# Picovoice/koala

Measured on AMD Instinct MI355X. Metric: 16 kHz frames/sec (batch 4096 streams per GPU), higher is better.
Workload: dtype bf16; 1 GPU; BASELINE configs[2]: batch=4096 streams/GPU x 64 frames/call, bf16 mask GEMMs on MFMA + fp32 FFT; streams_per_gpu=4096, frames_per_call=64, global_streams=4096, parallelism=streams sharded over 1 GPU(s), no data-path collective

## Files before the change

### koala_amd/csrc/kns_device.hpp

```cpp
#pragma once

#include <hip/hip_runtime.h>
#include <stdint.h>
#include <stdlib.h>

#include "kns_kernels.h"

namespace kns {

#ifdef KNS_TIMING
static __device__ unsigned long long g_kns_timing[8 * 16];
#define KNS_STAMP(i) do { if (blockIdx.x == 0 && (threadIdx.x & 63) == 0 && t == 5) g_kns_timing[(threadIdx.x >> 6) * 16 + (i)] = __builtin_amdgcn_s_memtime(); } while (0)
#define KNS_STAMP_AT(i, step) do { if (blockIdx.x == 0 && (threadIdx.x & 63) == 0 && t == (step)) g_kns_timing[(threadIdx.x >> 6) * 16 + (i)] = __builtin_amdgcn_s_memtime(); } while (0)
#define KNS_WSTAMP(i) do { if (dbg_stamp && (threadIdx.x & 63) == 0 && mt == m0 + 1) g_kns_timing[role * 16 + (i)] = __builtin_amdgcn_s_memtime(); } while (0)
#else
#define KNS_WSTAMP(i) do { } while (0)
#define KNS_STAMP(i) do { } while (0)
#define KNS_STAMP_AT(i, step) do { } while (0)
#endif

typedef float f32x4 __attribute__((ext_vector_type(4)));
typedef __bf16 bf16x8 __attribute__((ext_vector_type(8)));
typedef _Float16 f16x4 __attribute__((ext_vector_type(4)));

// ... 76 lines not shown
    __builtin_amdgcn_fence(__ATOMIC_RELEASE, "wavefront");
    __builtin_amdgcn_wave_barrier();
    __builtin_amdgcn_fence(__ATOMIC_ACQUIRE, "wavefront");
}


struct PF32 {
    static constexpr int kPrec = kFp32;
    static constexpr int KB = 16, EPL = 4, NPB = 1;
    static constexpr int NBH = 17;
    static constexpr bool kHoldA = false;
    static constexpr int kGruWaves = 1;
    typedef f32x4 frag_t;
    typedef f32x4 gi_t;
    typedef float elem_t;
    static __device__ __forceinline__ f32x4 mma(frag_t a, frag_t b, f32x4 c) {
        c = __builtin_amdgcn_mfma_f32_16x16x4f32(a[0], b[0], c, 0, 0, 0);
        c = __builtin_amdgcn_mfma_f32_16x16x4f32(a[1], b[1], c, 0, 0, 0);
        c = __builtin_amdgcn_mfma_f32_16x16x4f32(a[2], b[2], c, 0, 0, 0);
        c = __builtin_amdgcn_mfma_f32_16x16x4f32(a[3], b[3], c, 0, 0, 0);
        return c;
    }
    static __device__ __forceinline__ void mma2(frag_t a0, frag_t b0, f32x4 &c0, frag_t a1, frag_t b1, f32x4 &c1) {
#pragma unroll
        for (int q = 0; q < 4; ++q) {
            c0 = __builtin_amdgcn_mfma_f32_16x16x4f32(a0[q], b0[q], c0, 0, 0, 0);
            c1 = __builtin_amdgcn_mfma_f32_16x16x4f32(a1[q], b1[q], c1, 0, 0, 0);
        }
    }
    static __device__ __forceinline__ int off(int rc, int kk) { return pack_off_f32(rc, kk); }
    static __device__ __forceinline__ elem_t cvt(float v) { return v; }
    static __device__ __forceinline__ gi_t to_gi(f32x4 v) { return v; }
    static __device__ __forceinline__ f32x4 from_gi(gi_t v) { return v; }
};

struct PBF16 {
    static constexpr int kPrec = kBf16;
    static constexpr int KB = 32, EPL = 8, NPB = 2;
    static constexpr int NBH = 9;
    static constexpr bool kHoldA = true;
    static constexpr int kGruWaves = 1;
    typedef bf16x8 frag_t;
    typedef f16x4 gi_t;
    typedef uint16_t elem_t;
    static __device__ __forceinline__ f32x4 mma(frag_t a, frag_t b, f32x4 c) {
        return __builtin_amdgcn_mfma_f32_16x16x32_bf16(a, b, c, 0, 0, 0);
    }
    static __device__ __forceinline__ void mma2(frag_t a0, frag_t b0, f32x4 &c0, frag_t a1, frag_t b1, f32x4 &c1) {
        c0 = __builtin_amdgcn_mfma_f32_16x16x32_bf16(a0, b0, c0, 0, 0, 0);
        c1 = __builtin_amdgcn_mfma_f32_16x16x32_bf16(a1, b1, c1, 0, 0, 0);
    }
    static __device__ __forceinline__ int off(int rc, int kk) { return pack_off_bf16(rc, kk); }
    static __device__ __forceinline__ elem_t cvt(float v) { return f2bf(v); }
    static __device__ __forceinline__ gi_t to_gi(f32x4 v) { return __builtin_convertvector(v, gi_t); }
    static __device__ __forceinline__ f32x4 from_gi(gi_t v) {
        f32x4 r;
        r[0] = (float) v[0];
        r[1] = (float) v[1];
        r[2] = (float) v[2];
        r[3] = (float) v[3];
        return r;
    }
};


#ifdef KNS_CPX_PACKED
typedef float cpx __attribute__((ext_vector_type(2)));
__device__ __forceinline__ cpx cadd(cpx a, cpx b) { return a + b; }
__device__ __forceinline__ cpx csub(cpx a, cpx b) { return a - b; }
__device__ __forceinline__ cpx cmul(cpx a, cpx w) {
    const cpx t = cpx{a.y, a.y} * cpx{-w.y, w.x};
    return __builtin_elementwise_fma(cpx{a.x, a.x}, w, t);
}
#else
struct alignas(8) cpx {
    float x, y;
};
__device__ __forceinline__ cpx cadd(cpx a, cpx b) { return cpx{a.x + b.x, a.y + b.y}; }
__device__ __forceinline__ cpx csub(cpx a, cpx b) { return cpx{a.x - b.x, a.y - b.y}; }
__device__ __forceinline__ cpx cmul(cpx a, cpx w) {
    return cpx{__builtin_fmaf(a.x, w.x, a.y * -w.y), __builtin_fmaf(a.x, w.y, a.y * w.x)};
}
#endif

__device__ __forceinline__ void radix4(cpx (&v)[4]) {
    cpx a0 = cadd(v[0], v[2]), a1 = csub(v[0], v[2]), a2 = cadd(v[1], v[3]), d = csub(v[1], v[3]);
    cpx a3 = {d.y, -d.x};
    v[0] = cadd(a0, a2);
    v[1] = cadd(a1, a3);
    v[2] = csub(a0, a2);
    v[3] = csub(a1, a3);
}

constexpr int kFftRowBytes = 16 * 17 * 8;
constexpr int kFftWaveBytes = 4 * kFftRowBytes;
// ... 81 lines not shown
    return kns_sigmoid(x);
}
__device__ __forceinline__ float fast_tanh(float x) {
    return 1.0f - 2.0f * __builtin_amdgcn_rcpf(1.0f + __builtin_amdgcn_exp2f(x * 2.88539008177792681f));
}

typedef float f32x2 __attribute__((ext_vector_type(2)));
typedef __bf16 bf16x2 __attribute__((ext_vector_type(2)));

__device__ __forceinline__ __amdgpu_buffer_rsrc_t make_rsrc(const void *base, unsigned bytes) {
    return __builtin_amdgcn_make_buffer_rsrc((void *) base, 0, bytes, 0x00020000);
}
__device__ __forceinline__ bf16x8 buf_load_frag(__amdgpu_buffer_rsrc_t r, unsigned voff, unsigned soff) {
    return __builtin_bit_cast(bf16x8, __builtin_amdgcn_raw_buffer_load_b128(r, voff, soff, 0));
}
__device__ __forceinline__ void buf_store_frag(__amdgpu_buffer_rsrc_t r, unsigned voff, bf16x8 v) {
    typedef unsigned u32x4 __attribute__((ext_vector_type(4)));
    __builtin_amdgcn_raw_buffer_store_b128(__builtin_bit_cast(u32x4, v), r, voff, 0, 0);
}
__device__ __forceinline__ void buf_store_f32x4(__amdgpu_buffer_rsrc_t r, unsigned voff, f32x4 v) {
    typedef unsigned u32x4 __attribute__((ext_vector_type(4)));
    __builtin_amdgcn_raw_buffer_store_b128(__builtin_bit_cast(u32x4, v), r, voff, 0, 0);
}
__device__ __forceinline__ unsigned reset_rows(const unsigned *resets, int pitch, int mt, int t) {
    typedef const __attribute__((address_space(4))) unsigned *cptr_t;
    return __builtin_amdgcn_readfirstlane(((cptr_t) resets)[(size_t) mt * pitch + t]);
}

constexpr int kGiStreamAux = 2;
__device__ __forceinline__ void buf_store_gi(__amdgpu_buffer_rsrc_t r, unsigned voff, unsigned soff, f16x4 v) {
    typedef unsigned u32x2 __attribute__((ext_vector_type(2)));
    __builtin_amdgcn_raw_buffer_store_b64(__builtin_bit_cast(u32x2, v), r, voff, soff, kGiStreamAux);
}

__device__ __forceinline__ f32x2 gate_fma2(f32x2 a, f32x2 b, f32x2 c) {
#ifdef KNS_GATE_UNFUSED
    return a * b + c;
#else
    return __builtin_elementwise_fma(a, b, c);
#endif
}
__device__ __forceinline__ float gate_fma1(float a, float b, float c) {
#ifdef KNS_GATE_UNFUSED
    return a * b + c;
#else
    return __builtin_fmaf(a, b, c);
#endif
}
typedef _Float16 f16x2 __attribute__((ext_vector_type(2)));
__device__ __forceinline__ float opaque_one() {
    float one = 1.0f;
    asm("" : "+v"(one));
    return one;
}
template <int HI>
__device__ __forceinline__ float mix_add(unsigned x, float t, float one) {
    return __builtin_fmaf((float) __builtin_bit_cast(f16x2, x)[HI], one, t);
}
template <int HI>
__device__ __forceinline__ float mix_fma(float a, float b, unsigned x) {
    return __builtin_fmaf(a, b, (float) __builtin_bit_cast(f16x2, x)[HI]);
}

__device__ __forceinline__ float gate_rcp1p_exp2(float y) { return __builtin_amdgcn_rcpf(1.0f + __builtin_amdgcn_exp2f(y)); }
__device__ __forceinline__ f32x4 gate_block_bf16(const unsigned (&pr)[2], const unsigned (&pz)[2], const unsigned (&pn)[2],
                                                 const f32x4 &ar_, const f32x4 &az_, const f32x4 &an_, const f32x4 &hprev) {
// ... 35 lines not shown
```

### koala_amd/csrc/kns_gemm.hip

```cpp
#include "kns_device.hpp"

#include <type_traits>

namespace kns {


constexpr int kPF = 4;

template <class P, int OUT, int kGemmMT>
__global__ __launch_bounds__(256) void gemm_kernel(GemmArgs g) {
    extern __shared__ __attribute__((aligned(16))) char smem[];
    typedef typename P::frag_t frag_t;
    constexpr bool kApack = (OUT == kOutAPlain || OUT == kOutASigmoid);
    constexpr bool kSigmoid = (OUT == kOutMask || OUT == kOutASigmoid);
    constexpr int NU = kApack ? P::NPB : 1;

    const int tid = threadIdx.x, lane = tid & 63;
    const int wave = __builtin_amdgcn_readfirstlane(tid >> 6);
    const int nb = g.nb0 + g.taps * g.nb1;
    const int mt0 = blockIdx.x * kGemmMT;
    const int mcount = min(kGemmMT, g.mtiles - mt0);

    const int units = g.ntiles / NU;
    const int units_per_y = ceil_div(units, (int) gridDim.y);
// ... 50 lines not shown
                    for (int j = 0; j < NU; ++j) bc[j] = bq[p][j];
                    if (blk + kPF < nb)
#pragma unroll
                        for (int j = 0; j < NU; ++j) bq[p][j] = w[((size_t) (nt0 + j) * nb + blk + kPF) * 64 + lane];
#pragma unroll
                    for (int m = 0; m < kGemmMT; ++m) {
                        frag_t a = lds_f[(m * nb + blk) * 64 + lane];
#pragma unroll
                        for (int j = 0; j < NU; ++j) acc[j][m] = P::mma(a, bc[j], acc[j][m]);
                    }
                }
            }
        }

#pragma unroll
        for (int j = 0; j < NU; ++j) {
            const int nt = nt0 + j;
            const int col = nt * 16 + (lane & 15);
            const float bias = g.bias[col];
#pragma unroll
            for (int m = 0; m < kGemmMT; ++m) {
                f32x4 v = acc[j][m];
#pragma unroll
                for (int i = 0; i < 4; ++i) {
                    float x = v[i] + bias;
                    if (kSigmoid) x = head_sigmoid<P>(x);
                    if (kApack && col >= g.n_valid) x = 0.0f;
                    v[i] = x;
                }
                if (!kApack) {
                    if (m < mcount) {
                        const size_t idx = ((size_t) (mt0 + m) * g.ntiles + nt) * 64 + lane;
                        if (OUT == kOutGi)
                            ((typename P::gi_t *) g.out)[idx] = P::to_gi(v);
                        else if (P::kPrec == kBf16)
                            ((f16x4 *) g.out)[idx] = __builtin_convertvector(v, f16x4);
                        else
                            ((f32x4 *) g.out)[idx] = v;
                    }
                } else if (OUT == kOutASigmoid && g.pad_nb) {
                    if (m < mcount && col < g.n_valid) {
                        typename P::elem_t *dst = (typename P::elem_t *) g.out + ((size_t) (mt0 + m) * g.pad_nb + g.pad_blk) * 64 * P::EPL;
#pragma unroll
                        for (int i = 0; i < 4; ++i) dst[P::off((lane >> 4) * 4 + i, g.pad_kk0 + col)] = P::cvt(v[i]);
                    }
                } else {
                    typename P::elem_t *sc = (typename P::elem_t *) (scratch + m * 1024);
#pragma unroll
                    for (int i = 0; i < 4; ++i) sc[P::off((lane >> 4) * 4 + i, j * 16 + (lane & 15))] = P::cvt(v[i]);
                }
            }
        }
        if (kApack && !(OUT == kOutASigmoid && g.pad_nb)) {
            wave_lds_sync();
            const int out_nb = g.ntiles / NU;
            for (int m = 0; m < mcount; ++m) {
                uint4 word = ((const uint4 *) (scratch + m * 1024))[lane];
                ((uint4 *) g.out)[((size_t) (mt0 + m) * out_nb + u) * 64 + lane] = word;
            }
            wave_lds_sync();
        }
    }
}

constexpr int kWs2Waves = 8;
constexpr int kWs2Tiles = 4;

#ifndef WS2_NA
#define WS2_NA 2
#endif
constexpr int kWs2NA = WS2_NA;

template <int NB0, int kWs2Stage>
__global__ __launch_bounds__(64 * kWs2Waves, 2) void gemm_ws2_kernel(GemmArgs g) {
    typedef PBF16 P;
    typedef P::frag_t frag_t;
    constexpr int NB = P::NBH + NB0;
    __shared__ __attribute__((aligned(16))) char smem[2 * kWs2Stage * NB * 1024];
    frag_t *abuf = (frag_t *) smem;

    const int tid = threadIdx.x, lane = tid & 63;
    const int wave = __builtin_amdgcn_readfirstlane(tid >> 6);
    const int colq = lane & 15;
    const int bid = blockIdx.x;
    const int half = (bid >> 3) & 1;
    const int mgroup = (bid >> 4) * 8 + (bid & 7);
    const int mstride = (gridDim.x >> 1) * kWs2Stage;
    const int mlast = mgroup * kWs2Stage + ((g.mtiles - 1 - mgroup * kWs2Stage) / mstride) * mstride;
    const int nt_base = half ? 26 : 0, nt_count = half ? kGateTiles - 26 : 26;
    const frag_t *w = (const frag_t *) g.w;

    int nt[kWs2Tiles];
#pragma unroll
    for (int j = 0; j < kWs2Tiles; ++j) nt[j] = nt_base + (wave + kWs2Waves * j < nt_count ? wave + kWs2Waves * j : 0);
    const bool has4 = wave + kWs2Waves * 3 < nt_count;
    frag_t wr[kWs2Tiles][NB];
    float bias[kWs2Tiles];
#pragma unroll
    for (int j = 0; j < kWs2Tiles; ++j) {
#pragma unroll
        for (int blk = 0; blk < NB; ++blk) wr[j][blk] = w[((size_t) nt[j] * NB + blk) * 64 + lane];
        bias[j] = g.bias[nt[j] * 16 + colq];
    }

    constexpr int kStageBlocks = kWs2Stage * NB;
    constexpr int kFetch = (kStageBlocks + kWs2Waves - 1) / kWs2Waves;
    const unsigned lane16 = lane * 16u, lane8 = lane * 8u;
    unsigned foff[kFetch];
#pragma unroll
    for (int i = 0; i < kFetch; ++i) {
        const int idx = wave + kWs2Waves * i;
        const int m = idx / NB, blk = idx % NB;
        foff[i] = blk < NB0 ? (unsigned) (m * NB0 + blk) * 1024u : (unsigned) (m * P::NBH + (blk - NB0)) * 1024u;
    }
    auto fetch = [&](int i, int mt0) {
        const int blk = (wave + kWs2Waves * i) % NB;
        const __amdgpu_buffer_rsrc_t r =
            blk < NB0 ? make_rsrc((const frag_t *) g.a0 + (size_t) mt0 * NB0 * 64, kWs2Stage * (NB0 ? NB0 : 1) * 1024)
                      : make_rsrc((const frag_t *) g.a1 + (size_t) mt0 * P::NBH * 64, kWs2Stage * P::NBH * 1024);
        return buf_load_frag(r, lane16, foff[i]);
    };
#pragma unroll
    for (int i = 0; i < kFetch; ++i)
        if (wave + kWs2Waves * i < kStageBlocks) abuf[(wave + kWs2Waves * i) * 64 + lane] = fetch(i, mlast);
    __syncthreads();

    auto store_tile = [&](__amdgpu_buffer_rsrc_t out, int j, f32x4 v) {
#pragma unroll
        for (int i = 0; i < 4; ++i) v[i] = v[i] + bias[j];
        buf_store_gi(out, lane8, nt[j] * 512u, P::to_gi(v));
    };

    auto main_loop = [&](auto has4_tag) {
        constexpr bool kHas4 = decltype(has4_tag)::value;
        int cur = 0;
        for (int mt0 = mlast; mt0 >= 0; mt0 -= mstride) {
            const bool more = mt0 - mstride >= 0;
            frag_t stage[kFetch];
#pragma unroll
            for (int i = 0; i < kFetch; ++i)
                if (more && wave + kWs2Waves * i < kStageBlocks) stage[i] = fetch(i, mt0 - mstride);
            constexpr int MP = NB0 < 2 ? 2 : 1;
            static_assert(kWs2Stage % MP == 0, "m-tiles are processed MP at a time");
            const frag_t *ab = abuf + cur * kStageBlocks * 64;
#pragma unroll
            for (int m = 0; m < kWs2Stage; m += MP) {
                f32x4 acc[MP][kWs2Tiles];
                frag_t qa[MP][kWs2NA];
#pragma unroll
                for (int mm = 0; mm < MP; ++mm) {
#pragma unroll
                    for (int c = 0; c < kWs2Tiles; ++c) acc[mm][c] = f32x4{0.f, 0.f, 0.f, 0.f};
#pragma unroll
                    for (int p = 0; p < kWs2NA; ++p) qa[mm][p] = ab[((m + mm) * NB + p) * 64 + lane];
                }
                __builtin_amdgcn_sched_barrier(0);
#pragma unroll
                for (int blk = 0; blk < NB; ++blk) {
#pragma unroll
                    for (int c = 0; c < (kHas4 ? 4 : 3); ++c)
#pragma unroll
                        for (int mm = 0; mm < MP; ++mm) acc[mm][c] = P::mma(qa[mm][blk % kWs2NA], wr[c][blk], acc[mm][c]);
                    if (blk + kWs2NA < NB) {
#pragma unroll
                        for (int mm = 0; mm < MP; ++mm)
                            qa[mm][blk % kWs2NA] = ab[((m + mm) * NB + blk + kWs2NA) * 64 + lane];
                    }
                    __builtin_amdgcn_sched_barrier(0);
                }
                if (m == kWs2Stage - MP) {
#pragma unroll
                    for (int i = 0; i < kFetch; ++i)
                        if (more && wave + kWs2Waves * i < kStageBlocks)
                            abuf[((cur ^ 1) * kStageBlocks + wave + kWs2Waves * i) * 64 + lane] = stage[i];
                }
#pragma unroll
                for (int mm = 0; mm < MP; ++mm) {
                    const __amdgpu_buffer_rsrc_t out =
                        make_rsrc((P::gi_t *) g.out + (size_t) (mt0 + m + mm) * kGateTiles * 64, kGateTiles * 512);
#pragma unroll
                    for (int c = 0; c < (kHas4 ? 4 : 3); ++c) store_tile(out, c, acc[mm][c]);
                }
            }
            __syncthreads();
            cur ^= 1;
        }
    };
    if (has4)
        main_loop(std::true_type{});
    else
        main_loop(std::false_type{});
}

constexpr int kWsrStage = 2;

template <int OUT, int UW>
__global__ __launch_bounds__(512, 2) void gemm_wsr_kernel(GemmArgs g) {
    typedef PBF16 P;
    typedef P::frag_t frag_t;
    constexpr int NB = P::NBH;
    constexpr bool kApack = (OUT == kOutAPlain || OUT == kOutASigmoid);
    constexpr bool kSigmoid = (OUT == kOutMask || OUT == kOutASigmoid);
    constexpr int NU = kApack ? P::NPB : 1;
    __shared__ __attribute__((aligned(16))) char smem[2 * kWsrStage * NB * 1024 + 8 * 1024];
    frag_t *abuf = (frag_t *) smem;
    const int tid = threadIdx.x, lane = tid & 63;
    const int wave = __builtin_amdgcn_readfirstlane(tid >> 6);
    char *scratch = smem + 2 * kWsrStage * NB * 1024 + wave * 1024;
    const int colq = lane & 15;
    const int units = g.ntiles / NU;
    const frag_t *w = (const frag_t *) g.w;

    int unit[UW];
    bool live[UW];
    frag_t wr[UW * NU][NB];
    float bias[UW * NU];
#pragma unroll
    for (int q = 0; q < UW; ++q) {
        live[q] = wave + 8 * q < units;
        unit[q] = live[q] ? wave + 8 * q : 0;
#pragma unroll
        for (int j = 0; j < NU; ++j) {
            const int nt = unit[q] * NU + j;
#pragma unroll
// ... 386 lines not shown
        launch_gemm_mt<P, 2>(a, s);
    else
        launch_gemm_mt<P, 1>(a, s);
}

void launch_gemm(const GemmArgs &a, hipStream_t s) {
    const bool no_ws = (a.dev & kDevGemmGeneric) != 0;
    if (a.precision == kBf16 && a.out_kind == kOutGi && a.ntiles == kGateTiles && a.nb1 == PBF16::NBH && a.nb0 <= 2 && a.taps == 1 &&
        a.mtiles >= 256 && !no_ws) {
        GemmArgs m = a;
        m.mtiles = a.mtiles / 256 * 256;
        const int wgs = a.grid >= 16 && a.grid < 256 ? (a.grid / 16 >= 8 ? 128 : a.grid / 16 >= 4 ? 64 : a.grid / 16 >= 2 ? 32 : 16) : 256;
        const dim3 grid(wgs), block(64 * kWs2Waves);
        if (m.mtiles % 512 == 0) {
            if (a.nb0 == 0)
                hipLaunchKernelGGL((gemm_ws2_kernel<0, 4>), grid, block, 0, s, m);
            else if (a.nb0 == 1)
                hipLaunchKernelGGL((gemm_ws2_kernel<1, 4>), grid, block, 0, s, m);
            else
                hipLaunchKernelGGL((gemm_ws2_kernel<2, 4>), grid, block, 0, s, m);
        } else {
            if (a.nb0 == 0)
                hipLaunchKernelGGL((gemm_ws2_kernel<0, 2>), grid, block, 0, s, m);
            else if (a.nb0 == 1)
                hipLaunchKernelGGL((gemm_ws2_kernel<1, 2>), grid, block, 0, s, m);
            else
                hipLaunchKernelGGL((gemm_ws2_kernel<2, 2>), grid, block, 0, s, m);
        }
        if (a.mtiles > m.mtiles) {
            GemmArgs t = a;
            t.mtiles = a.mtiles - m.mtiles;
            if (a.a0) t.a0 = (const char *) a.a0 + (size_t) m.mtiles * a.nb0 * 1024;
            t.a1 = (const char *) a.a1 + (size_t) m.mtiles * a.nb1 * 1024;
            t.out = (char *) a.out + (size_t) m.mtiles * kGateTiles * 64 * sizeof(PBF16::gi_t);
            launch_gemm_p<PBF16>(t, s);
        }
        return;
    }
    const bool no_wsr = (a.dev & kDevGemmNoWsr) != 0;
    if (a.precision == kBf16 && a.nb0 == 0 && a.nb1 == PBF16::NBH && a.taps == kF5Taps && a.out_kind == kOutAPlain && a.ntiles == 18 &&
        a.tap_stride % ((size_t) a.nb1 * 1024) == 0 && !no_wsr) {
        const int mtb = (int) (a.tap_stride / ((size_t) a.nb1 * 1024));
        const int T = mtb > 0 ? a.mtiles / mtb : 0;
        if (T >= 8 && a.mtiles == T * mtb) {
            int nseg = 1;
            while (mtb * nseg < 256 && T / (nseg * 2) >= 16) nseg *= 2;
            int seglen = (T + nseg - 1) / nseg;
            seglen = (seglen + kF5P - 1) / kF5P * kF5P;
            nseg = (T + seglen - 1) / seglen;
            const int jobs = mtb * nseg;
            allow_dynamic_lds(gemm_front5_kernel, kF5LdsBytes);
            hipLaunchKernelGGL(gemm_front5_kernel, dim3((jobs + 7) / 8 * 24), dim3(64 * kF5Waves), kF5LdsBytes, s, a, mtb, T, seglen);
            return;
        }
        if (a.mtiles <= 1024) {
            allow_dynamic_lds(gemm_front5_t1_kernel, kF5tLdsBytes);
            hipLaunchKernelGGL(gemm_front5_t1_kernel, dim3((a.mtiles + 7) / 8 * 24), dim3(64 * kF5Waves), kF5tLdsBytes, s, a);
            return;
        }
    }
    if (a.precision == kBf16 && a.nb0 == 0 && a.nb1 == PBF16::NBH && a.taps == 1 && a.mtiles >= 512 && !no_wsr) {
        const dim3 grid(a.grid >= 16 && a.grid < 256 ? a.grid : 256), block(512);
        if (a.out_kind == kOutAPlain && a.ntiles <= 32) {
            hipLaunchKernelGGL((gemm_wsr_kernel<kOutAPlain, 2>), grid, block, 0, s, a);
            return;
        }
        if (a.out_kind == kOutASigmoid && a.pad_nb && a.ntiles != 2) {
// ... 28 lines not shown
```

### koala_amd/csrc/kns_gru.hip

```cpp
#include "kns_device.hpp"

namespace kns {


template <class P, int W, bool kResets = false>
__global__ __launch_bounds__(64 * W, W / 4) void gru_kernel(GruArgs g) {
    typedef typename P::frag_t frag_t;
    typedef typename P::elem_t elem_t;
    constexpr int NBH = P::NBH;
    constexpr int TPW = (kUnitTiles + W - 1) / W;
    __shared__ __attribute__((aligned(16))) char hbuf[2][NBH * 1024];

    const int tid = threadIdx.x, lane = tid & 63;
    const int wave = __builtin_amdgcn_readfirstlane(tid >> 6);
    const int mt = blockIdx.x;
    const int colq = lane & 15, rowq = (lane >> 4) * 4;

    f32x4 hreg[TPW];
#pragma unroll
    for (int q = 0; q < TPW; ++q) {
        const int u = wave + W * q;
        hreg[q] = f32x4{0.f, 0.f, 0.f, 0.f};
        if (u < kUnitTiles) hreg[q] = ((const f32x4 *) g.hstate_in)[((size_t) mt * kUnitTiles + u) * 64 + lane];
    }
// ... 26 lines not shown
    const frag_t *whh = (const frag_t *) g.whh;
    int cur = 0;
    for (int t = 0; t < g.T; ++t) {
        const frag_t *ha = (const frag_t *) hbuf[cur];
        if (t > 0) {
            frag_t *hs = (frag_t *) g.hseq + ((size_t) (t - 1) * g.mtiles + mt) * NBH * 64;
            for (int blk = wave; blk < NBH; blk += W) hs[blk * 64 + lane] = ha[blk * 64 + lane];
        }
        if (kResets) {
            const unsigned rm = reset_rows(g.resets, g.rs_pitch, mt, g.rs_t0 + t);
            if (rm) {
                __syncthreads();
#pragma unroll
                for (int q = 0; q < TPW; ++q) {
                    const int u = wave + W * q;
                    if (u < kUnitTiles) {
                        const int k = u * 16 + colq;
                        elem_t *dst = (elem_t *) hbuf[cur] + (k / P::KB) * 64 * P::EPL;
#pragma unroll
                        for (int i = 0; i < 4; ++i) {
                            hreg[q][i] = (rm >> (rowq + i)) & 1u ? 0.0f : hreg[q][i];
                            dst[P::off(rowq + i, k % P::KB)] = operand_of(hreg[q][i], u);
                        }
                    }
                }
                __syncthreads();
            }
        }
        const typename P::gi_t *gi = (const typename P::gi_t *) g.gi + ((size_t) t * g.mtiles + mt) * kGateTiles * 64;
#pragma unroll
        for (int q = 0; q < TPW; ++q) {
            const int u = wave + W * q;
            if (u < kUnitTiles) {
                typename P::gi_t gir = gi[(u * 3 + 0) * 64 + lane];
                typename P::gi_t giz = gi[(u * 3 + 1) * 64 + lane];
                typename P::gi_t gin = gi[(u * 3 + 2) * 64 + lane];
                const float br = g.bhh[(u * 3 + 0) * 16 + colq];
                const float bz = g.bhh[(u * 3 + 1) * 16 + colq];
                const float bn = g.bhh[(u * 3 + 2) * 16 + colq];
                f32x4 acc[3];
#pragma unroll
                for (int gt = 0; gt < 3; ++gt) acc[gt] = f32x4{0.f, 0.f, 0.f, 0.f};
                const frag_t *wu = whh + (size_t) u * 3 * NBH * 64 + lane;
                constexpr int kAhead = 4;
                frag_t bq[kAhead][3];
#pragma unroll
                for (int p = 0; p < kAhead; ++p)
#pragma unroll
                    for (int gt = 0; gt < 3; ++gt) bq[p][gt] = wu[(gt * NBH + (p < NBH ? p : NBH - 1)) * 64];
#pragma nounroll
                for (int blk = 0; blk < NBH; ++blk) {
                    const frag_t ab = ha[blk * 64 + lane];
                    frag_t bc[3];
#pragma unroll
                    for (int gt = 0; gt < 3; ++gt) {
                        bc[gt] = bq[0][gt];
#pragma unroll
                        for (int p = 0; p + 1 < kAhead; ++p) bq[p][gt] = bq[p + 1][gt];
                    }
                    const int nb = blk + kAhead < NBH ? blk + kAhead : NBH - 1;
#pragma unroll
                    for (int gt = 0; gt < 3; ++gt) bq[kAhead - 1][gt] = wu[(gt * NBH + nb) * 64];
#pragma unroll
                    for (int gt = 0; gt < 3; ++gt) acc[gt] = P::mma(ab, bc[gt], acc[gt]);
                }
                f32x4 ir = P::from_gi(gir), iz = P::from_gi(giz), in = P::from_gi(gin);
                const int k = u * 16 + colq;
                elem_t *dst = (elem_t *) hbuf[cur ^ 1] + (k / P::KB) * 64 * P::EPL;
                if (P::kPrec == kBf16) {
// ... 471 lines not shown
#pragma unroll
        for (int p = 0; p <= D; ++p) aq[p] = ha[p * 64 + lane];
    }
#pragma unroll
    for (int p = 0; p < kQ; ++p)
        if (kFirstLds + p < N) qb[p] = wl[p * 64 + lane];
    if (kChain) qc = w16[0];
    if (D == 0) aq[0] = ha[lane];
#pragma unroll
    for (int i = 0; i < N; ++i) {
        const int blk = i / 3;
        if (i % 3 == 0 && blk > 0 && blk + D < NB) aq[(blk + D) % (D + 1)] = ha[(blk + D) * 64 + lane];
        const bf16x8 a = aq[blk % (D + 1)];
        bf16x8 b;
        if (i < kFirstLds) {
            b = wreg[i < kNReg ? i : 0];
        } else {
            const int j = i - kFirstLds;
            b = qb[j % kQ];
            if (i + kQ < N) qb[j % kQ] = wl[(j + kQ) * 64 + lane];
        }
        acc[i % 3] = PBF16::mma(a, b, acc[i % 3]);
        if (kChain && i % 3 == 2) {
            const bf16x8 c = qc;
            if (blk + 1 < NB) qc = w16[(blk + 1) * kChainStride * 64];
            *a16 = PBF16::mma(a, c, *a16);
        }
    }
}

__device__ __forceinline__ f16x4 buf_load_gi(__amdgpu_buffer_rsrc_t r, unsigned voff, unsigned soff) {
    return __builtin_bit_cast(f16x4, __builtin_amdgcn_raw_buffer_load_b64(r, voff, soff, kGiStreamAux));
}

template <bool kYHead, bool kResets = false>
__global__ __launch_bounds__(64 * kR8Waves, 2) void gru_resident8_kernel(GruArgs g) {
    typedef PBF16 P;
    typedef P::frag_t frag_t;
    constexpr int NBH = P::NBH;
    constexpr int kApf = kYHead ? R8_APF_Y : kResets ? R8_APF_R : R8_APF;
    constexpr bool kPublish = !kYHead;
    __shared__ __attribute__((aligned(16))) char smem[kR8Lds + 3 * 1024 + 16 + (kYHead ? kR8HeadLds : 0)];
    frag_t *wlh = (frag_t *) (smem + kR8Lds + 3 * 1024 + 16);
    char *hbuf0 = smem, *hbuf1 = smem + NBH * 1024;
    frag_t *wl1 = (frag_t *) (smem + 2 * NBH * 1024);
    frag_t *wl16 = (frag_t *) (smem + 2 * NBH * 1024 + kR8Waves * (kR8LdsFrags0 + kR8LdsFrags1) * 1024);
    f32x4 *acc16 = (f32x4 *) (smem + kR8Lds);

    const int tid = threadIdx.x, lane = tid & 63;
    const int wave = __builtin_amdgcn_readfirstlane(tid >> 6);
    const int mt = blockIdx.x;
    const int colq = lane & 15, rowq = (lane >> 4) * 4;
    const frag_t *whh = (const frag_t *) g.whh;
    const int u0 = wave, u1 = wave + 8, u2 = 16;
#ifndef R8_CHAIN0
#define R8_CHAIN0 1
#endif
#ifndef R8_ROW0
#define R8_ROW0 0
#endif
    const int g16 = wave - R8_CHAIN0;
    const bool c16 = wave >= R8_CHAIN0 && wave <= R8_CHAIN0 + 2;
    const bool q16 = wave >= R8_ROW0 && wave < R8_ROW0 + 4;
    const unsigned flag16 = (unsigned) (uintptr_t) (smem + kR8Lds + 3 * 1024);

    typedef const __attribute__((address_space(1))) void *gptr_t;
    typedef __attribute__((address_space(3))) void *lptr_t;
    frag_t *wl0w = wl1 + wave * (kR8LdsFrags0 + kR8LdsFrags1) * 64, *wl1w = wl0w + kR8LdsFrags0 * 64;
#pragma unroll
    for (int i = kR8RegFrags0; i < 27; ++i)
        __builtin_amdgcn_global_load_lds((gptr_t) (whh + ((size_t) (u0 * 3 + i % 3) * NBH + i / 3) * 64 + lane),
                                         (lptr_t) (wl0w + (i - kR8RegFrags0) * 64), 16, 0, 0);
#pragma unroll
    for (int i = kR8RegFrags1; i < 27; ++i)
        __builtin_amdgcn_global_load_lds((gptr_t) (whh + ((size_t) (u1 * 3 + i % 3) * NBH + i / 3) * 64 + lane),
                                         (lptr_t) (wl1w + (i - kR8RegFrags1) * 64), 16, 0, 0);
    for (int i = wave; i < 27; i += kR8Waves)
        __builtin_amdgcn_global_load_lds((gptr_t) (whh + ((size_t) (u2 * 3 + i % 3) * NBH + i / 3) * 64 + lane),
                                         (lptr_t) (wl16 + i * 64), 16, 0, 0);
    if (kYHead) {
        for (int i = wave; i < NBH; i += kR8Waves)
            __builtin_amdgcn_global_load_lds((gptr_t) ((const frag_t *) g.yw + (size_t) i * 64 + lane), (lptr_t) (wlh + i * 64), 16, 0, 0);
    }
    const float ybias = kYHead ? g.yb[colq] : 0.0f;
    frag_t w0[kR8RegFrags0], w1[kR8RegFrags1];
#pragma unroll
    for (int i = 0; i < kR8RegFrags0; ++i) w0[i] = whh[((size_t) (u0 * 3 + i % 3) * NBH + i / 3) * 64 + lane];
#pragma unroll
    for (int i = 0; i < kR8RegFrags1; ++i) w1[i] = whh[((size_t) (u1 * 3 + i % 3) * NBH + i / 3) * 64 + lane];
    f32x4 hreg[2];
    hreg[0] = ((const f32x4 *) g.hstate_in)[((size_t) mt * kUnitTiles + u0) * 64 + lane];
    hreg[1] = ((const f32x4 *) g.hstate_in)[((size_t) mt * kUnitTiles + u1) * 64 + lane];
    const int e16 = q16 ? wave - R8_ROW0 : 0;
    float h16 = g.hstate_in[(((size_t) mt * kUnitTiles + u2) * 64 + lane) * 4 + e16];
    P::gi_t gi[2][3], gi16[3];
    {
        const P::gi_t *gp = (const P::gi_t *) g.gi + (size_t) mt * kGateTiles * 64;
#pragma unroll
        for (int gt = 0; gt < 3; ++gt) {
            gi[0][gt] = gp[(u0 * 3 + gt) * 64 + lane];
            gi[1][gt] = gp[(u1 * 3 + gt) * 64 + lane];
            gi16[gt] = gp[(u2 * 3 + gt) * 64 + lane];
        }
    }
    for (int i = tid; i < 2 * NBH * 64; i += 64 * kR8Waves) ((uint4 *) smem)[i] = uint4{0, 0, 0, 0};
    if (tid < 4) ((int *) (smem + kR8Lds + 3 * 1024))[tid] = 0;
    __syncthreads();
    if (tid < 64) {
        const int k = kBiasK0 + ((tid >> 4) & 1);
        ((uint16_t *) ((tid >> 5) ? hbuf1 : hbuf0))[(k / P::KB) * 64 * P::EPL + P::off(tid & 15, k % P::KB)] = (uint16_t) kBf16One;
    }
    auto put_h = [&](char *buf, int u, const f32x4 &h) {
        const int k = u * 16 + colq;
        uint16_t *dst = (uint16_t *) buf + (k / P::KB) * 64 * P::EPL + P::off(rowq, k % P::KB);
        const uint32_t lo = __builtin_bit_cast(uint32_t, __builtin_convertvector(f32x2{h[0], h[1]}, bf16x2));
        const uint32_t hi = __builtin_bit_cast(uint32_t, __builtin_convertvector(f32x2{h[2], h[3]}, bf16x2));
        dst[0] = (uint16_t) lo;
        dst[8] = (uint16_t) (lo >> 16);
        dst[16] = (uint16_t) hi;
        dst[24] = (uint16_t) (hi >> 16);
    };
    auto put_h16 = [&](char *buf, float h) {
        const int k = u2 * 16 + colq;
        uint16_t *dst = (uint16_t *) buf + (k / P::KB) * 64 * P::EPL + P::off(rowq + e16, k % P::KB);
        dst[0] = colq == 15 ? (uint16_t) kBf16One : f2bf(h);
    };
    put_h(hbuf0, u0, hreg[0]);
    put_h(hbuf0, u1, hreg[1]);
    if (q16) put_h16(hbuf0, h16);
    __syncthreads();

    const unsigned lane8 = lane * 8u;
    const size_t hs_stride = (size_t) g.mtiles * NBH * 1024, gi_stride = (size_t) g.mtiles * kGateTiles * 512;
    const char *hs_base = kPublish ? (const char *) g.hseq + (size_t) mt * NBH * 1024 : nullptr;
    const char *gn_base = (const char *) g.gi + (size_t) mt * kGateTiles * 512 + (g.T > 1 ? gi_stride : 0);
    auto publish = [&](const frag_t *src, const char *slot_base) {
        const __amdgpu_buffer_rsrc_t hs = make_rsrc(slot_base, NBH * 1024);
        const unsigned i0 = wave * 64 + lane, i1 = 8 * 64 + wave * 8 + (lane & 7);
        const frag_t x0 = src[i0];
        buf_store_frag(hs, i0 * 16u, x0);
        const frag_t x1 = src[i1];
        buf_store_frag(hs, lane < 8 ? i1 * 16u : 0x7fffff00u, x1);
    };
    const size_t y_frame_bytes = (size_t) g.mtiles * g.y_nb * 1024;
    auto emit_y = [&](const f32x4 &ya, int frame) {
        uint16_t *dst = (uint16_t *) ((char *) g.yout + (size_t) frame * y_frame_bytes + ((size_t) mt * g.y_nb + g.y_blk) * 1024);
        if (colq < g.yvalid) {
#pragma unroll
            for (int i = 0; i < 4; ++i) dst[P::off(rowq + i, g.y_kk0 + colq)] = P::cvt(head_sigmoid<PBF16>(ya[i] + ybias));
        }
    };
    for (int t = 0; t < g.T; ++t) {
        KNS_STAMP(0);
        KNS_STAMP_AT(9, 8);
        KNS_STAMP_AT(10, 24);
        char *hc = (t & 1) ? hbuf1 : hbuf0;
        char *hn = (t & 1) ? hbuf0 : hbuf1;
        const frag_t *ha = (const frag_t *) hc;
        if (kPublish) publish(ha, hs_base);
        bool reset_step = false;
        if (kResets) {
            const unsigned rm = reset_rows(g.resets, g.rs_pitch, mt, g.rs_t0 + t);
            reset_step = rm != 0;
            if (reset_step) {
                if (kYHead && wave == 0 && t > 0) {
                    f32x4 ya = f32x4{0.f, 0.f, 0.f, 0.f};
#pragma nounroll
                    for (int blk = 0; blk < NBH; ++blk) ya = P::mma(ha[blk * 64 + lane], wlh[blk * 64 + lane], ya);
                    emit_y(ya, t - 1);
                }
                __syncthreads();
            }
            const unsigned rb = rm >> rowq;
#pragma unroll
            for (int q = 0; q < 2; ++q)
#pragma unroll
                for (int i = 0; i < 4; ++i) hreg[q][i] = (rb >> i) & 1u ? 0.0f : hreg[q][i];
            h16 = (rb >> e16) & 1u ? 0.0f : h16;
            if (reset_step) {
                put_h(hc, u0, hreg[0]);
                put_h(hc, u1, hreg[1]);
                if (q16) put_h16(hc, h16);
                __syncthreads();
            }
        }
        const __amdgpu_buffer_rsrc_t gnext = make_rsrc(gn_base, kGateTiles * 512);
        if (kPublish) hs_base += t > 0 ? hs_stride : 0;
        gn_base += t + 2 < g.T ? gi_stride : 0;

        auto gates = [&](const int q, f32x4 (&acc)[3]) {
            typedef unsigned u32x2 __attribute__((ext_vector_type(2)));
            const u32x2 vr = __builtin_bit_cast(u32x2, gi[q][0]), vz = __builtin_bit_cast(u32x2, gi[q][1]),
                        vn = __builtin_bit_cast(u32x2, gi[q][2]);
            const unsigned pr[2] = {vr[0], vr[1]}, pz[2] = {vz[0], vz[1]}, pn[2] = {vn[0], vn[1]};
            const int u = q ? u1 : u0;
#pragma unroll
            for (int gt = 0; gt < 3; ++gt) gi[q][gt] = buf_load_gi(gnext, lane8, (u * 3 + gt) * 512u);
            const f32x4 hnew = gate_block_bf16(pr, pz, pn, acc[0], acc[1], acc[2], hreg[q]);
            hreg[q] = hnew;
            put_h(hn, u, hnew);
        };
        auto acc_init = [&](f32x4 (&acc)[3], const int) {
#pragma unroll
            for (int gt = 0; gt < 3; ++gt) acc[gt] = f32x4{0.f, 0.f, 0.f, 0.f};
        };
        KNS_STAMP(1);
        f32x4 acc[3];
        acc_init(acc, u0);
        if (kYHead && wave == 0) {
            f32x4 ya = f32x4{0.f, 0.f, 0.f, 0.f};
            r8_tile_mma<kR8RegFrags0, R8C_Q, kR8RegFrags0, true, 1, kApf>(acc, ha, w0, wl0w, lane, &ya, wlh + lane);
            if (!reset_step) emit_y(ya, t > 0 ? t - 1 : 0);
        } else {
            r8_tile_mma<kR8RegFrags0, R8C_Q, kR8RegFrags0, false, 3, kApf>(acc, ha, w0, wl0w, lane);
        }
        KNS_STAMP(2);
        gates(0, acc);
        KNS_STAMP(3);
        acc_init(acc, u1);
        if (c16) {
            f32x4 a16 = f32x4{0.f, 0.f, 0.f, 0.f};
            r8_tile_mma<kR8RegFrags1, R8C_Q, kR8RegFrags1, true, 3, kApf>(acc, ha, w1, wl1w, lane, &a16, wl16 + g16 * 64 + lane);
            acc16[g16 * 64 + lane] = a16;
            asm volatile("ds_write_b32 %0, %1" ::"v"(flag16 + g16 * 4), "v"(t + 1) : "memory");
        } else {
            r8_tile_mma<kR8RegFrags1, 3, kR8RegFrags1, false, 3, kApf>(acc, ha, w1, wl1w, lane);
        }
        KNS_STAMP(4);
        gates(1, acc);
        KNS_STAMP(5);
        KNS_STAMP(6);
        {
            const float xr = (float) gi16[0][e16], xz = (float) gi16[1][e16], xn = (float) gi16[2][e16];
#pragma unroll
            for (int gt = 0; gt < 3; ++gt) gi16[gt] = buf_load_gi(gnext, lane8, (u2 * 3 + gt) * 512u);
            if (q16) {
                typedef int i32x4 __attribute__((ext_vector_type(4)));
                i32x4 f;
                do {
                    asm volatile("ds_read_b128 %0, %1\n\ts_waitcnt lgkmcnt(0)" : "=v"(f) : "v"(flag16) : "memory");
                } while (__builtin_amdgcn_readfirstlane(f[0] + f[1] + f[2]) != 3 * (t + 1));
                const float ar = ((const float *) acc16)[(0 * 64 + lane) * 4 + e16];
                const float az = ((const float *) acc16)[(1 * 64 + lane) * 4 + e16];
                const float an = ((const float *) acc16)[(2 * 64 + lane) * 4 + e16];
                h16 = gate_elem_bf16(xr, xz, xn, ar, az, an, h16);
                put_h16(hn, h16);
            }
        }
        KNS_STAMP(7);
        __syncthreads();
        KNS_STAMP(8);
    }
    if (kYHead && wave == 0) {
        const frag_t *hl = (const frag_t *) ((g.T & 1) ? hbuf1 : hbuf0);
        f32x4 ya = f32x4{0.f, 0.f, 0.f, 0.f};
#pragma unroll
        for (int blk = 0; blk < NBH; ++blk) ya = P::mma(hl[blk * 64 + lane], wlh[blk * 64 + lane], ya);
        emit_y(ya, g.T - 1);
    }
    if (kPublish)
        publish((const frag_t *) ((g.T & 1) ? hbuf1 : hbuf0), (const char *) g.hseq + ((size_t) (g.T - 1) * g.mtiles + mt) * NBH * 1024);
    ((f32x4 *) g.hstate_out)[((size_t) mt * kUnitTiles + u0) * 64 + lane] = hreg[0];
    ((f32x4 *) g.hstate_out)[((size_t) mt * kUnitTiles + u1) * 64 + lane] = hreg[1];
    int lane_o = lane;
    if (kYHead) asm volatile("" : "+v"(lane_o));
    if (q16) g.hstate_out[(((size_t) mt * kUnitTiles + u2) * 64 + lane_o) * 4 + e16] = h16;
}

// ... 26 lines not shown
```

### koala_amd/csrc/kns_layout.h

```cpp
#pragma once

#include <stdint.h>

#if defined(__HIPCC__)
#define KNS_HD __host__ __device__ inline
#else
#define KNS_HD inline
#endif

namespace kns {

constexpr int kFrame = 256;
constexpr int kNfft = 512;
constexpr int kBins = 257;
constexpr int kHidden = 271;
constexpr int kUnitTiles = 17;
constexpr int kGateTiles = 3 * kUnitTiles;
constexpr int kStages = 4;
constexpr int kMaskTiles = 17;
constexpr int kGruLayers = 2 * kStages;
constexpr float kGateScaleRZ = -1.44269504088896341f;
constexpr float kGateScaleN = 2.88539008177792681f;
constexpr int kBiasK0 = kHidden;
constexpr unsigned kBf16One = 0x3f80u;
constexpr int kYPadMax = 7;
constexpr int kMaxFrontTaps = 5;

enum Precision { kFp32 = 0, kBf16 = 1 };

struct PrecInfo {
    int kb;
    int epl;
    int esz;
    int npb;
    int gisz;
};

KNS_HD PrecInfo prec_info(int precision) {
    return precision == kBf16 ? PrecInfo{32, 8, 2, 2, 8} : PrecInfo{16, 4, 4, 1, 16};
}

KNS_HD int ceil_div(int a, int b) { return (a + b - 1) / b; }

KNS_HD int pack_off_bf16(int rc, int kk) { return (rc + 16 * (kk >> 3)) * 8 + (kk & 7); }
KNS_HD int pack_off_f32(int rc, int kk) { return (rc + 16 * (kk & 3)) * 4 + (kk >> 2); }
KNS_HD int pack_off(int precision, int rc, int kk) {
    return precision == kBf16 ? pack_off_bf16(rc, kk) : pack_off_f32(rc, kk);
}

KNS_HD int cpack_off(int row, int col) { return ((row >> 2) * 16 + col) * 4 + (row & 3); }

}
```

Measured before the change: 104.9 million frames/s.

## Interleave GRU input-gate tiles into paired 16-byte slots for wider loads/stores

Changes the bf16 gate-input (gi) buffer layout so that pairs of gate tiles belonging to the same wave's units are interleaved per lane into 1024-byte slots. The GEMM epilogue then writes two tiles with one 128-bit buffer store, and the resident GRU kernel loads r/z/n gate inputs with three 128-bit loads instead of six 64-bit loads. This touches the GEMM tile assignment per wave, the epilogue and the GRU prefetch, aiming to cut memory instruction count and improve coalescing on the latency-critical recurrent path. It adds complex index math and a special case for the 17th unit tile, with a risk of layout mismatches between producer and consumer.

```diff
diff --git a/koala_amd/csrc/kns_device.hpp b/koala_amd/csrc/kns_device.hpp
--- a/koala_amd/csrc/kns_device.hpp
+++ b/koala_amd/csrc/kns_device.hpp
@@ -132,6 +132,7 @@
     static __device__ __forceinline__ elem_t cvt(float v) { return v; }
     static __device__ __forceinline__ gi_t to_gi(f32x4 v) { return v; }
     static __device__ __forceinline__ f32x4 from_gi(gi_t v) { return v; }
+    static __device__ __forceinline__ int gi_index(int nt, int lane) { return nt * 64 + lane; }
 };
 
 struct PBF16 {
@@ -161,6 +162,7 @@
         r[3] = (float) v[3];
         return r;
     }
+    static __device__ __forceinline__ int gi_index(int nt, int lane) { return (int) (gi_cell_off(nt, lane) / sizeof(gi_t)); }
 };
 
 
@@ -308,6 +310,15 @@
     typedef unsigned u32x2 __attribute__((ext_vector_type(2)));
     __builtin_amdgcn_raw_buffer_store_b64(__builtin_bit_cast(u32x2, v), r, voff, soff, kGiStreamAux);
 }
+typedef unsigned gi_slot_t __attribute__((ext_vector_type(4)));
+__device__ __forceinline__ void buf_store_gi_slot(__amdgpu_buffer_rsrc_t r, unsigned voff, f16x4 lo, f16x4 hi) {
+    typedef unsigned u32x2 __attribute__((ext_vector_type(2)));
+    const u32x2 a = __builtin_bit_cast(u32x2, lo), b = __builtin_bit_cast(u32x2, hi);
+    __builtin_amdgcn_raw_buffer_store_b128(gi_slot_t{a[0], a[1], b[0], b[1]}, r, voff, 0, kGiStreamAux);
+}
+__device__ __forceinline__ gi_slot_t buf_load_gi_slot(__amdgpu_buffer_rsrc_t r, unsigned voff, unsigned soff) {
+    return __builtin_amdgcn_raw_buffer_load_b128(r, voff, soff, kGiStreamAux);
+}
 
 __device__ __forceinline__ f32x2 gate_fma2(f32x2 a, f32x2 b, f32x2 c) {
 #ifdef KNS_GATE_UNFUSED
diff --git a/koala_amd/csrc/kns_gemm.hip b/koala_amd/csrc/kns_gemm.hip
--- a/koala_amd/csrc/kns_gemm.hip
+++ b/koala_amd/csrc/kns_gemm.hip
@@ -106,7 +106,7 @@
                     if (m < mcount) {
                         const size_t idx = ((size_t) (mt0 + m) * g.ntiles + nt) * 64 + lane;
                         if (OUT == kOutGi)
-                            ((typename P::gi_t *) g.out)[idx] = P::to_gi(v);
+                            ((typename P::gi_t *) g.out)[(size_t) (mt0 + m) * g.ntiles * 64 + P::gi_index(nt, lane)] = P::to_gi(v);
                         else if (P::kPrec == kBf16)
                             ((f16x4 *) g.out)[idx] = __builtin_convertvector(v, f16x4);
                         else
@@ -161,13 +161,19 @@
     const int mgroup = (bid >> 4) * 8 + (bid & 7);
     const int mstride = (gridDim.x >> 1) * kWs2Stage;
     const int mlast = mgroup * kWs2Stage + ((g.mtiles - 1 - mgroup * kWs2Stage) / mstride) * mstride;
-    const int nt_base = half ? 26 : 0, nt_count = half ? kGateTiles - 26 : 26;
     const frag_t *w = (const frag_t *) g.w;
 
+    static constexpr signed char kSlotA[2][8] = {{0, 2, 4, 5, 6, 8, 9, 11}, {12, 14, 15, 17, 18, 20, 21, 23}};
+    static constexpr signed char kSingleSlot[2][8] = {{-1, -1, -1, -1, 7, 7, 10, 10}, {-1, -1, 16, 16, 19, 19, 22, 22}};
+    static constexpr signed char kSingleSub[2][8] = {{-1, -1, 0, 1, 0, 1, 0, 1}, {-1, 2, 0, 1, 0, 1, 0, 1}};
+    const int slot0 = kSlotA[half][wave];
+    const int ssub = kSingleSub[half][wave], sslot = kSingleSlot[half][wave];
+    const int ntw = ssub < 0 ? 4 : 3;
     int nt[kWs2Tiles];
-#pragma unroll
-    for (int j = 0; j < kWs2Tiles; ++j) nt[j] = nt_base + (wave + kWs2Waves * j < nt_count ? wave + kWs2Waves * j : 0);
-    const bool has4 = wave + kWs2Waves * 3 < nt_count;
+    nt[0] = gi_slot_tile(slot0, 0);
+    nt[1] = gi_slot_tile(slot0, 1);
+    nt[2] = ntw == 4 ? gi_slot_tile(slot0 + 1, 0) : sslot >= 0 ? gi_slot_tile(sslot, ssub) : 3 * 16 + ssub;
+    nt[3] = ntw == 4 ? gi_slot_tile(slot0 + 1, 1) : nt[0];
     frag_t wr[kWs2Tiles][NB];
     float bias[kWs2Tiles];
 #pragma unroll
@@ -179,7 +185,7 @@
 
     constexpr int kStageBlocks = kWs2Stage * NB;
     constexpr int kFetch = (kStageBlocks + kWs2Waves - 1) / kWs2Waves;
-    const unsigned lane16 = lane * 16u, lane8 = lane * 8u;
+    const unsigned lane16 = lane * 16u;
     unsigned foff[kFetch];
 #pragma unroll
     for (int i = 0; i < kFetch; ++i) {
@@ -199,14 +205,26 @@
         if (wave + kWs2Waves * i < kStageBlocks) abuf[(wave + kWs2Waves * i) * 64 + lane] = fetch(i, mlast);
     __syncthreads();
 
-    auto store_tile = [&](__amdgpu_buffer_rsrc_t out, int j, f32x4 v) {
-#pragma unroll
-        for (int i = 0; i < 4; ++i) v[i] = v[i] + bias[j];
-        buf_store_gi(out, lane8, nt[j] * 512u, P::to_gi(v));
-    };
-
-    auto main_loop = [&](auto has4_tag) {
-        constexpr bool kHas4 = decltype(has4_tag)::value;
+    const unsigned slot_base = gi_cell_off(nt[0], 0);
+    const unsigned single_base = gi_cell_off(nt[2], 0);
+    const unsigned single_voff = gi_cell_off(nt[2], lane) - single_base;
+    auto add_bias = [](f32x4 v, float b) {
+#pragma unroll
+        for (int i = 0; i < 4; ++i) v[i] = v[i] + b;
+        return v;
+    };
+    auto store_slot = [&](const char *out_mt, int k, f32x4 v0, f32x4 v1) {
+        v0 = add_bias(v0, bias[2 * k]);
+        v1 = add_bias(v1, bias[2 * k + 1]);
+        buf_store_gi_slot(make_rsrc(out_mt + slot_base + k * 1024u, 1024u), lane16, P::to_gi(v0), P::to_gi(v1));
+    };
+    auto store_single = [&](const char *out_mt, f32x4 v) {
+        v = add_bias(v, bias[2]);
+        buf_store_gi(make_rsrc(out_mt + single_base, sslot >= 0 ? 1024u - 8u : (unsigned) kGiTileBytes), single_voff, 0, P::to_gi(v));
+    };
+
+    auto main_loop = [&](auto ntw_tag) {
+        constexpr int kNtw = decltype(ntw_tag)::value;
         int cur = 0;
         for (int mt0 = mlast; mt0 >= 0; mt0 -= mstride) {
             const bool more = mt0 - mstride >= 0;
@@ -232,7 +250,7 @@
 #pragma unroll
                 for (int blk = 0; blk < NB; ++blk) {
 #pragma unroll
-                    for (int c = 0; c < (kHas4 ? 4 : 3); ++c)
+                    for (int c = 0; c < kNtw; ++c)
 #pragma unroll
                         for (int mm = 0; mm < MP; ++mm) acc[mm][c] = P::mma(qa[mm][blk % kWs2NA], wr[c][blk], acc[mm][c]);
                     if (blk + kWs2NA < NB) {
@@ -250,20 +268,20 @@
                 }
 #pragma unroll
                 for (int mm = 0; mm < MP; ++mm) {
-                    const __amdgpu_buffer_rsrc_t out =
-                        make_rsrc((P::gi_t *) g.out + (size_t) (mt0 + m + mm) * kGateTiles * 64, kGateTiles * 512);
-#pragma unroll
-                    for (int c = 0; c < (kHas4 ? 4 : 3); ++c) store_tile(out, c, acc[mm][c]);
+                    const char *out = (const char *) g.out + (size_t) (mt0 + m + mm) * kGiMtileBytes;
+                    store_slot(out, 0, acc[mm][0], acc[mm][1]);
+                    if (kNtw == 4) store_slot(out, 1, acc[mm][2], acc[mm][3]);
+                    if (kNtw == 3) store_single(out, acc[mm][2]);
                 }
             }
             __syncthreads();
             cur ^= 1;
         }
     };
-    if (has4)
-        main_loop(std::true_type{});
+    if (ntw == 4)
+        main_loop(std::integral_constant<int, 4>{});
     else
-        main_loop(std::false_type{});
+        main_loop(std::integral_constant<int, 3>{});
 }
 
 constexpr int kWsrStage = 2;
@@ -716,7 +734,7 @@
             t.mtiles = a.mtiles - m.mtiles;
             if (a.a0) t.a0 = (const char *) a.a0 + (size_t) m.mtiles * a.nb0 * 1024;
             t.a1 = (const char *) a.a1 + (size_t) m.mtiles * a.nb1 * 1024;
-            t.out = (char *) a.out + (size_t) m.mtiles * kGateTiles * 64 * sizeof(PBF16::gi_t);
+            t.out = (char *) a.out + (size_t) m.mtiles * kGiMtileBytes;
             launch_gemm_p<PBF16>(t, s);
         }
         return;
diff --git a/koala_amd/csrc/kns_gru.hip b/koala_amd/csrc/kns_gru.hip
--- a/koala_amd/csrc/kns_gru.hip
+++ b/koala_amd/csrc/kns_gru.hip
@@ -82,9 +82,9 @@
         for (int q = 0; q < TPW; ++q) {
             const int u = wave + W * q;
             if (u < kUnitTiles) {
-                typename P::gi_t gir = gi[(u * 3 + 0) * 64 + lane];
-                typename P::gi_t giz = gi[(u * 3 + 1) * 64 + lane];
-                typename P::gi_t gin = gi[(u * 3 + 2) * 64 + lane];
+                typename P::gi_t gir = gi[P::gi_index(u * 3 + 0, lane)];
+                typename P::gi_t giz = gi[P::gi_index(u * 3 + 1, lane)];
+                typename P::gi_t gin = gi[P::gi_index(u * 3 + 2, lane)];
                 const float br = g.bhh[(u * 3 + 0) * 16 + colq];
                 const float bz = g.bhh[(u * 3 + 1) * 16 + colq];
                 const float bn = g.bhh[(u * 3 + 2) * 16 + colq];
@@ -622,6 +622,9 @@
 __device__ __forceinline__ f16x4 buf_load_gi(__amdgpu_buffer_rsrc_t r, unsigned voff, unsigned soff) {
     return __builtin_bit_cast(f16x4, __builtin_amdgcn_raw_buffer_load_b64(r, voff, soff, kGiStreamAux));
 }
+__device__ __forceinline__ __amdgpu_buffer_rsrc_t gi_mtile_rsrc(const void *mtile, bool with16) {
+    return make_rsrc(mtile, with16 ? kGiMtileBytes : kGiSlots * 1024);
+}
 
 template <bool kYHead, bool kResets = false>
 __global__ __launch_bounds__(64 * kR8Waves, 2) void gru_resident8_kernel(GruArgs g) {
@@ -683,15 +686,16 @@
     hreg[1] = ((const f32x4 *) g.hstate_in)[((size_t) mt * kUnitTiles + u1) * 64 + lane];
     const int e16 = q16 ? wave - R8_ROW0 : 0;
     float h16 = g.hstate_in[(((size_t) mt * kUnitTiles + u2) * 64 + lane) * 4 + e16];
-    P::gi_t gi[2][3], gi16[3];
+    const unsigned gs_voff = gi_cell_off(u0 * 3, lane);
+    const unsigned g16_voff = gi_cell_off(u2 * 3, lane);
+    gi_slot_t gs[3];
+    P::gi_t gi16[3];
     {
-        const P::gi_t *gp = (const P::gi_t *) g.gi + (size_t) mt * kGateTiles * 64;
-#pragma unroll
-        for (int gt = 0; gt < 3; ++gt) {
-            gi[0][gt] = gp[(u0 * 3 + gt) * 64 + lane];
-            gi[1][gt] = gp[(u1 * 3 + gt) * 64 + lane];
-            gi16[gt] = gp[(u2 * 3 + gt) * 64 + lane];
-        }
+        const __amdgpu_buffer_rsrc_t g0 = gi_mtile_rsrc((const char *) g.gi + (size_t) mt * kGiMtileBytes, q16);
+#pragma unroll
+        for (int k = 0; k < 3; ++k) gs[k] = buf_load_gi_slot(g0, gs_voff, k * 1024u);
+#pragma unroll
+        for (int gt = 0; gt < 3; ++gt) gi16[gt] = buf_load_gi(g0, g16_voff, gt * kGiTileBytes);
     }
     for (int i = tid; i < 2 * NBH * 64; i += 64 * kR8Waves) ((uint4 *) smem)[i] = uint4{0, 0, 0, 0};
     if (tid < 4) ((int *) (smem + kR8Lds + 3 * 1024))[tid] = 0;
@@ -720,10 +724,9 @@
     if (q16) put_h16(hbuf0, h16);
     __syncthreads();
 
-    const unsigned lane8 = lane * 8u;
-    const size_t hs_stride = (size_t) g.mtiles * NBH * 1024, gi_stride = (size_t) g.mtiles * kGateTiles * 512;
+    const size_t hs_stride = (size_t) g.mtiles * NBH * 1024, gi_stride = (size_t) g.mtiles * kGiMtileBytes;
     const char *hs_base = kPublish ? (const char *) g.hseq + (size_t) mt * NBH * 1024 : nullptr;
-    const char *gn_base = (const char *) g.gi + (size_t) mt * kGateTiles * 512 + (g.T > 1 ? gi_stride : 0);
+    const char *gn_base = (const char *) g.gi + (size_t) mt * kGiMtileBytes + (g.T > 1 ? gi_stride : 0);
     auto publish = [&](const frag_t *src, const char *slot_base) {
         const __amdgpu_buffer_rsrc_t hs = make_rsrc(slot_base, NBH * 1024);
         const unsigned i0 = wave * 64 + lane, i1 = 8 * 64 + wave * 8 + (lane & 7);
@@ -774,18 +777,21 @@
                 __syncthreads();
             }
         }
-        const __amdgpu_buffer_rsrc_t gnext = make_rsrc(gn_base, kGateTiles * 512);
+        const __amdgpu_buffer_rsrc_t gnext = gi_mtile_rsrc(gn_base, q16);
         if (kPublish) hs_base += t > 0 ? hs_stride : 0;
         gn_base += t + 2 < g.T ? gi_stride : 0;
 
         auto gates = [&](const int q, f32x4 (&acc)[3]) {
-            typedef unsigned u32x2 __attribute__((ext_vector_type(2)));
-            const u32x2 vr = __builtin_bit_cast(u32x2, gi[q][0]), vz = __builtin_bit_cast(u32x2, gi[q][1]),
-                        vn = __builtin_bit_cast(u32x2, gi[q][2]);
-            const unsigned pr[2] = {vr[0], vr[1]}, pz[2] = {vz[0], vz[1]}, pn[2] = {vn[0], vn[1]};
+            const unsigned pr[2] = {q ? gs[1][2] : gs[0][0], q ? gs[1][3] : gs[0][1]};
+            const unsigned pz[2] = {q ? gs[2][0] : gs[0][2], q ? gs[2][1] : gs[0][3]};
+            const unsigned pn[2] = {q ? gs[2][2] : gs[1][0], q ? gs[2][3] : gs[1][1]};
             const int u = q ? u1 : u0;
-#pragma unroll
-            for (int gt = 0; gt < 3; ++gt) gi[q][gt] = buf_load_gi(gnext, lane8, (u * 3 + gt) * 512u);
+            if (q == 0) {
+                gs[0] = buf_load_gi_slot(gnext, gs_voff, 0);
+            } else {
+                gs[1] = buf_load_gi_slot(gnext, gs_voff, 1024u);
+                gs[2] = buf_load_gi_slot(gnext, gs_voff, 2048u);
+            }
             const f32x4 hnew = gate_block_bf16(pr, pz, pn, acc[0], acc[1], acc[2], hreg[q]);
             hreg[q] = hnew;
             put_h(hn, u, hnew);
@@ -823,7 +829,7 @@
         {
             const float xr = (float) gi16[0][e16], xz = (float) gi16[1][e16], xn = (float) gi16[2][e16];
 #pragma unroll
-            for (int gt = 0; gt < 3; ++gt) gi16[gt] = buf_load_gi(gnext, lane8, (u2 * 3 + gt) * 512u);
+            for (int gt = 0; gt < 3; ++gt) gi16[gt] = buf_load_gi(gnext, g16_voff, gt * kGiTileBytes);
             if (q16) {
                 typedef int i32x4 __attribute__((ext_vector_type(4)));
                 i32x4 f;
diff --git a/koala_amd/csrc/kns_layout.h b/koala_amd/csrc/kns_layout.h
--- a/koala_amd/csrc/kns_layout.h
+++ b/koala_amd/csrc/kns_layout.h
@@ -50,4 +50,18 @@
 
 KNS_HD int cpack_off(int row, int col) { return ((row >> 2) * 16 + col) * 4 + (row & 3); }
 
+constexpr int kGiSlots = 24;
+constexpr int kGiTileBytes = 512;
+constexpr int kGiMtileBytes = kGateTiles * kGiTileBytes;
+KNS_HD int gi_slot_tile(int slot, int e) {
+    const int w = slot / 3, s = 2 * (slot - 3 * w) + e;
+    return 3 * (w + 8 * (s / 3)) + s % 3;
 }
+KNS_HD unsigned gi_cell_off(int nt, int lane) {
+    const int u = nt / 3, g = nt - 3 * u;
+    if (u >= 16) return (unsigned) (nt * kGiTileBytes + lane * 8);
+    const int w = u & 7, s = 3 * (u >> 3) + g;
+    return (unsigned) ((3 * w + (s >> 1)) * 1024 + lane * 16 + (s & 1) * 8);
+}
+
+}
```

Result: no change. 105.3 million frames/s (median of 4 runs) (+0.3%).
